# houkensjtu/taichi-2d-vof

Hardware: AMD Instinct MI355X
Metric: cell-updates/sec (whole node), 4096x4096 fp64 dam-break (higher is better)
Workload: dtype f64; 1 GPU; 4096x4096 -ic 1 f64, dt 4e-06, 10 Jacobi sweeps/step, single strip; nx=4096, ny=4096, jacobi_iters=10, exchange=none, tm_choice=1, step_schedule=k_tm batch graphs (k_transport + the next step's k_momentum as one kernel), handle_warm_steps=19

## Files before the change

### taichi-2d-vof_amd/csrc/kernels/jacobi_pair.h

```cpp
#pragma once
#include "jacobi.h"

namespace vof {

template <typename T, int V>
struct JpRing {
  static constexpr int W = 64 * V, NR = 8;
  T p[NR][W], b[NR][W];
  int hit;
};
template <typename T, int V>
__device__ __forceinline__ void jp_put(T (&row)[64 * V], int lane, const T (&c)[V]) {
  Pack<T, V> k;
#pragma unroll
  for (int q = 0; q < V; ++q) k.v[q] = c[q];
  *reinterpret_cast<Pack<T, V>*>(&row[lane * V]) = k;
}
template <typename T, int V>
__device__ __forceinline__ void jp_get(T (&c)[V], const T (&row)[64 * V], int lane) {
  const Pack<T, V> k = *reinterpret_cast<const Pack<T, V>*>(&row[lane * V]);
#pragma unroll
  for (int q = 0; q < V; ++q) c[q] = k.v[q];
}

template <typename T, int V, int TS, bool BS, int ROLE, int ABL = 0>
__device__ __forceinline__ void jacobi_pair_march(const Geom& g, const Consts<T>& c, const T* __restrict__ p,
                                                  const T* __restrict__ rhs, T* __restrict__ pn, JpRing<T, V>& lds,
                                                  int c0, int lane, int ra, int rb, WaveTimer& wt) {
  if constexpr ((ROLE == 0 && !(ABL & ABL_PRIO0)) || (ROLE == 1 && (ABL & ABL_PRIO1))) __builtin_amdgcn_s_setprio(1);
  constexpr int W = 64 * V;
  constexpr int H = ((2 * TS + V - 1) / V) * V;
  const int j0 = c0 + lane * V;
  const int nx = g.nx, ny = g.ny;
  const int jlo = c0 + H > 1 ? c0 + H : 1;
  const int jhi = c0 + W - H - 1 < ny ? c0 + W - H - 1 : ny;
  const int64_t pitch = g.pitch;
  T cj[V], apI[V], yI[V];
#pragma unroll
  for (int q = 0; q < V; ++q) {
    const int j = j0 + q;
    const T an = j != ny ? c.dyi2 : (T)0.0, as_ = j != 1 ? c.dyi2 : (T)0.0;
    cj[q] = (j >= 1 && j <= ny) ? c.dxi2 : (T)0.0;
    apI[q] = (T)-1.0 * (c.dxi2 + c.dxi2 + an + as_);
    yI[q] = (T)1 / apI[q];
    if (j < 1 || j > ny) yI[q] = (T)0;
  }
  auto rowptr = [&](const T* base, int r) {
    if constexpr ((ABL & ABL_FIXED_ROW) != 0) r = ra;
    const int rc = r < g.row_lo ? g.row_lo : (r > g.row_hi ? g.row_hi : r);
    return base + (size_t)(rc - g.row_lo) * (size_t)pitch + (size_t)(g.col0 + j0);
  };
  auto to_products = [&](T (&row)[V], int r) {
    const bool rowok = r >= 1 && r <= nx;
#pragma unroll
    for (int q = 0; q < V; ++q) row[q] = (rowok ? cj[q] : (T)0.0) * row[q];
  };
  T ring[TS][3][V];
  T rq[6][V];
#pragma unroll
  for (int s = 0; s < TS; ++s)
#pragma unroll
    for (int k = 0; k < 3; ++k)
#pragma unroll
      for (int q = 0; q < V; ++q) ring[s][k][q] = (T)0;
#pragma unroll
  for (int k = 0; k < 6; ++k)
#pragma unroll
    for (int q = 0; q < V; ++q) rq[k][q] = (T)0;
  const int t0 = ra - TS + 2, t1 = rb + TS;
  if constexpr (ROLE == 0) {
    load_c<T, V>(ring[0][0], rowptr(p, t0 - 2));
    load_c<T, V>(ring[0][1], rowptr(p, t0 - 1));
    load_c<T, V>(ring[0][2], rowptr(p, t0));
    load_s<T, V>(rq[0], rowptr(rhs, t0 - 1));
  } else {
    for (int k = 0; k < 2 * TS + 2; ++k) wt.barrier();
    jp_get<T, V>(ring[0][0], lds.p[(t0 - 2) & 7], lane);
    jp_get<T, V>(ring[0][1], lds.p[(t0 - 1) & 7], lane);
    jp_get<T, V>(ring[0][2], lds.p[t0 & 7], lane);
    jp_get<T, V>(rq[0], lds.b[(t0 - 1) & 7], lane);
  }
  to_products(ring[0][0], t0 - 2);
  to_products(ring[0][1], t0 - 1);
  const T* const pn_tile = pn + (int64_t)(g.col0 + c0);
  const int voff_st = (j0 >= jlo && j0 + V - 1 <= jhi) ? lane * (int)(V * sizeof(T)) : kBufSkip;
  const T* const p_tile = p + (int64_t)(g.col0 + c0);
  const T* const rhs_tile = rhs + ((int64_t)(g.col0 + c0) - pitch);
  const int voff_ld = lane * (int)(V * sizeof(T));
  int soff = 0;
  auto sub = [&](auto uc, auto fc, int t) {
    constexpr int U = decltype(uc)::value;
    constexpr bool FAST = decltype(fc)::value != 0;
    constexpr int kM = U % 3, kC = (U + 1) % 3, kE = (U + 2) % 3;
    T carry[V];
    if constexpr (ROLE == 1 && (ABL & ABL_IDLE1)) { wt.barrier(); return; }
    if constexpr (ROLE == 0) jp_put<T, V>(lds.b[(t - 1) & 7], lane, rq[U % 6]);
    if constexpr (ROLE == 0 && (ABL & ABL_PASS0)) {
      const int io = t - TS;
      if (io >= ra && io <= rb) jp_put<T, V>(lds.p[io & 7], lane, ring[0][kC]);
      if (t < t1) {
        load_c<T, V>(ring[0][kM], rowptr(p, t + 1));
        load_s<T, V>(rq[(U + 1) % 6], rowptr(rhs, t));
      }
      wt.barrier();
      return;
    }
    if constexpr (FAST) {
#pragma unroll
      for (int q = 0; q < V; ++q) ring[0][kE][q] = cj[q] * ring[0][kE][q];
    } else {
      to_products(ring[0][kE], t);
    }
#pragma unroll
    for (int s = 1; s <= TS; ++s) {
      const int i = t - s;
      const T sl = lane_up_z(ring[s - 1][kC][V - 1]);
      const T sr = lane_dn_z(ring[s - 1][kC][0]);
      if (s > 1) {
        const T coef = (FAST || (i + 1 >= 1 && i + 1 <= nx)) ? c.dxi2 : (T)0.0;
#pragma unroll
        for (int q = 0; q < V; ++q) ring[s - 1][kE][q] = coef * carry[q];
      }
      if (!FAST && s > 1 && t < ra - TS + 2 * s) continue;
      const bool edge = !FAST && ((i == 1) || (i == nx));
      const int slot = ((U + 1 - s) % 6 + 6) % 6;
      T num[V];
#pragma unroll
      for (int q = 0; q < V; ++q) {
        const T N = q == V - 1 ? sr : ring[s - 1][kC][q + 1];
        const T S = q == 0 ? sl : ring[s - 1][kC][q - 1];
        num[q] = rq[slot][q] - ring[s - 1][kE][q] - ring[s - 1][kM][q] - N - S;
      }
      if (edge) {
        const T ae = i != nx ? c.dxi2 : (T)0.0;
        const T aw = i != 1 ? c.dxi2 : (T)0.0;
#pragma unroll
        for (int q = 0; q < V; ++q) {
          int j = j0 + q;
          asm volatile("" : "+v"(j));
          const T an = j != ny ? c.dyi2 : (T)0.0, as_ = j != 1 ? c.dyi2 : (T)0.0;
          const T ap = (T)-1.0 * (ae + aw + an + as_);
          T o = div_by_const<T>(num[q], ap, (T)1.0 / ap);
          if (j < 1 || j > ny) o = (T)0;
          carry[q] = o;
        }
      } else {
        div_by_const_v<T, V, false, ColdFlagLds>(carry, num, apI, yI, ColdFlagLds{&lds.hit});
      }
      if (s == 1) {
        if constexpr (FAST) {
          if constexpr (ROLE == 0) {
            load_buf<T, V>(ring[0][kM], p_tile, voff_ld, soff, false);
            load_buf<T, V>(rq[(U + 1) % 6], rhs_tile, voff_ld, soff, true);
            if constexpr ((ABL & ABL_FIXED_ROW) == 0) soff += (int)(pitch * (int64_t)sizeof(T));
          } else {
            jp_get<T, V>(ring[0][kM], lds.p[(t + 1) & 7], lane);
            jp_get<T, V>(rq[(U + 1) % 6], lds.b[t & 7], lane);
          }
        } else if (t < t1) {
          if constexpr (ROLE == 0) {
            load_c<T, V>(ring[0][kM], rowptr(p, t + 1));
            load_s<T, V>(rq[(U + 1) % 6], rowptr(rhs, t));
          } else {
            jp_get<T, V>(ring[0][kM], lds.p[(t + 1) & 7], lane);
            jp_get<T, V>(rq[(U + 1) % 6], lds.b[t & 7], lane);
          }
        }
      }
    }
    const int io = t - TS;
    if constexpr (ROLE == 0) {
      if (FAST || (io >= ra && io <= rb)) jp_put<T, V>(lds.p[io & 7], lane, carry);
    } else if constexpr ((ABL & ABL_NO_STORE) != 0) {
      asm volatile("" :: "v"(carry[0]), "v"(carry[V - 1]));
    } else if constexpr (BS) {
      if constexpr (FAST) {
        store_buf_nt<T, V>(pn_tile, voff_st, soff, carry);
        soff += (int)(pitch * (int64_t)sizeof(T));
      } else {
        store_buf_nt<T, V>(pn_tile, (io >= ra && io <= rb) ? voff_st : kBufSkip,
                           (io >= ra && io <= rb) ? (int)((int64_t)(io - g.row_lo) * pitch * (int64_t)sizeof(T)) : 0, carry);
      }
    } else if (FAST || (io >= ra && io <= rb)) {
      store_s<T, V>(pn + at(g, io, j0), carry, j0, jlo, jhi);
    }
    wt.barrier();
  };
  auto imax3 = [](int a, int b, int d) { return a > b ? (a > d ? a : d) : (b > d ? b : d); };
  auto imin3 = [](int a, int b, int d) { return a < b ? (a < d ? a : d) : (b < d ? b : d); };
  const int fast_lo = imax3(ra + TS, TS + 2, g.row_lo + TS);
  const int fast_hi = imin3(nx - 1, t1 - 1, g.row_hi - 1);
  int t = t0;
  bool done = false;
  for (int phase = 0; phase < 2; ++phase) {
    for (; !done && t <= t1 && (phase == 1 || t < fast_lo || t + 5 > fast_hi); t += 6) {
      sub(IC<0>{}, IC<0>{}, t);
      if (t + 1 > t1) { done = true; break; }
      sub(IC<1>{}, IC<0>{}, t + 1);
      if (t + 2 > t1) { done = true; break; }
      sub(IC<2>{}, IC<0>{}, t + 2);
      if (t + 3 > t1) { done = true; break; }
      sub(IC<3>{}, IC<0>{}, t + 3);
      if (t + 4 > t1) { done = true; break; }
      sub(IC<4>{}, IC<0>{}, t + 4);
      if (t + 5 > t1) { done = true; break; }
      sub(IC<5>{}, IC<0>{}, t + 5);
    }
    if (BS && phase == 0 && !done && t <= t1 && t >= fast_lo && t + 5 <= fast_hi) {
      soff = (int)((int64_t)((ROLE == 0 ? t + 1 : t - TS) - g.row_lo) * pitch * (int64_t)sizeof(T));
      for (; t + 5 <= fast_hi; t += 6) {
        sub(IC<0>{}, IC<1>{}, t);
        sub(IC<1>{}, IC<1>{}, t + 1);
        sub(IC<2>{}, IC<1>{}, t + 2);
        sub(IC<3>{}, IC<1>{}, t + 3);
        sub(IC<4>{}, IC<1>{}, t + 4);
        sub(IC<5>{}, IC<1>{}, t + 5);
      }
    }
  }
  if constexpr (ROLE == 0) { wt.barrier(); wt.barrier(); }
}

template <typename T, int V, int TS, bool BS, int ABL = 0>
__global__ __launch_bounds__(128) __attribute__((amdgpu_waves_per_eu(4))) void k_jacobi_pair(Geom g, Consts<T> c, const T* __restrict__ p,
                                                     const T* __restrict__ rhs, T* __restrict__ pn, int R, int ntt,
                                                     TbPlan tp, int first, int last) {
  constexpr int W = 64 * V;
  constexpr int H = ((2 * TS + V - 1) / V) * V;
  constexpr int STRIDE = W - 2 * H;
  __shared__ __attribute__((aligned(16))) JpRing<T, V> lds;
  WaveTimer wt_(WT_JACOBI_PAIR);
  if (last < first) { first = g.ilo; last = g.ihi; }
  const int pair = (int)blockIdx.x;
  const int role = __builtin_amdgcn_readfirstlane(threadIdx.x >> 6);
  const int lane = threadIdx.x & 63;
  int upair;
  upair = xcd_grouped_block(pair, (int)gridDim.x);
  int tj = upair % ntt, ra = first + (upair / ntt) * R, rb = ra + R - 1;
  bool planned = false;
  if (tp.masks != nullptr) {
    const unsigned long long* pl = tp.plan;
    if (pl[0] == plan_key(tp)) {
      const unsigned long long e = pl[1 + pair];
      tj = (int)(e & 0xffull);
      ra = (int)((e >> 8) & 0xfffffffull);
      rb = (int)((e >> 36) & 0xfffffffull);
      planned = true;
    }
  }
  tj = __builtin_amdgcn_readfirstlane(tj);
  ra = __builtin_amdgcn_readfirstlane(ra);
  rb = __builtin_amdgcn_readfirstlane(rb);
  if (planned && rb < ra) return;
  if (planned && ra < first) ra = first;
  if (ra > last) return;
  if (rb > last) rb = last;
  if (rb < ra) return;
  const int c0 = 1 - H + tj * STRIDE;
  if (threadIdx.x == 0) lds.hit = 0;
  __syncthreads();
  if (role == 0) {
    jacobi_pair_march<T, V, TS, BS, 0, ABL>(g, c, p, rhs, pn, lds, c0, lane, ra - TS, rb + TS, wt_);
  } else {
    jacobi_pair_march<T, V, TS, BS, 1, ABL>(g, c, p, rhs, pn, lds, c0, lane, ra, rb, wt_);
  }
  if (tp.masks != nullptr) {
    __syncthreads();
    if (threadIdx.x == 0 && lds.hit != 0) {
      for (int b = tb_band_of(g, ra < g.ilo ? g.ilo : ra); b <= tb_band_of(g, rb > g.ihi ? g.ihi : rb); ++b)
        atomicOr(tp.masks + tb_word(tp.par ^ 1, b, tj), 1ull << (tj & 63));
    }
  }
}

}
```

### taichi-2d-vof_amd/csrc/runtime/context.h

```cpp
#pragma once
#include <vector>

#include <float.h>
#include <hip/hip_runtime.h>
#include <hip/hip_ext.h>
#include <dlfcn.h>

#include <cmath>
#include <cstdio>
#include <cstdlib>
#include <cstring>
#include <map>
#include <new>

#include "../../../include/vof2d.h"
#include "../vof2d_kernels.h"

using namespace vof;

struct RcclId { char internal[VOF_COMM_ID_BYTES]; };

namespace {

enum FieldId { fF = 0, fF2, fU, fV, fP, fPT, fUS, fVS, fMX, fMY, fKAPPA, fRHO, fNU, fRHS, NFIELDS };
// ... 162 lines not shown
  double* mg_sc = nullptr;
  int mg_nu = 2;
  int mg_levels = -1;
  int mg_graph = 1;
  void* mg_key[3] = {nullptr, nullptr, nullptr};
  int mg_coarse_block = 0;
  double* mg_rec = nullptr;
  void* step_mg_key[NFIELDS] = {};
  int step_mg_cycles = 0, step_mg_crit = 0;
  double* diag_part = nullptr;
  double* diag_rows = nullptr;
  int64_t diag_cap = 0;
  int rows_override = 0;
  int tb = 5;
  int tb_rows = 0;
  int mom_rows = 0;
  int tb_general = 0;
  int tb_adapt = 1;
  unsigned long long* d_tbmask = nullptr;
  long tbplan_cap = 0;
  int fctx_rows = 0;
  int fctx_corr_rows = 0;
  int fuse_transport = 1;
  int band_rows = 4;
  int buf_stores = 7;
  int virtual_ghosts = 1;
  void* f_home = nullptr;
  void* us_home = nullptr;
  void* p_home = nullptr;
  int phase_graph_ori = 0;
  GraphCache graphs;
  static constexpr int kStepBatches = GraphCache::kStepBatches;
  static constexpr int kTuneBatch = 1;
  int step_batch[kStepBatches] = {16, 8, 2};
  int fuse_tm = -1;
  double gas_share = -1.0;
  unsigned long long* h_gas = nullptr;
  hipEvent_t ev_gas = nullptr;
  bool gas_pending = false;
  bool tm_broken = false;
  bool alt_dirty = false;
  bool ahead = false;
  bool tm_rhs_alt = false;
  int64_t tm_chained = 0;
  int jpair = 1;
  int jpair_rows = 0;
  int solve_pairs = -1;
  int pair_slow10 = 32;
  int tb_slow10 = 20;
  int pair_vec4 = 0;
  bool jpair_active = false;
  bool jpair_captured = false;
  int64_t pair_launches = 0;
  TuneState tune;
  int64_t tm_steps = 0;
  int tm_rows = 0;
  int halves = -1;
  std::vector<hipStream_t> chain_streams;
  bool halves_captured[kStepBatches] = {};
  int64_t halves_steps = 0;
  std::vector<hipEvent_t> hev;
  bool batching = true;
  int next_phase = 0;
  bool f_ghosts_dirty = true;
  bool uv_ghosts_dirty = false;
  bool ghosts_virtual = false;
  void* vis = nullptr;
  size_t vis_bytes = 0;
  static constexpr int kMaxTimed = 96;
  hipEvent_t tev[2 * kMaxTimed] = {};
  int timed = -1;
  int tkid[kMaxTimed];
  double prof_sum_ms[24] = {};
  long prof_cnt[24] = {};
  std::map<const void*, long> occ_cache;
  void* comm = nullptr;
  hipStream_t cstream = nullptr;
  hipEvent_t ev_ready = nullptr, ev_done = nullptr;
  hipEvent_t ev_fork[3] = {nullptr, nullptr, nullptr};
  int xchg5_graph = 1;
  int xchg_pair = 1;
  int xchg_graph = 1;
  int64_t xchg_steps = 0;
  int64_t xchg_graph_steps = 0;
  double* d_red = nullptr;
  int comm_rank = 0, comm_world = 1;
  int peer_lo = -1, peer_hi = -1;
  char err[512];
};

namespace {

#define HIPCHK(h, call)                                                                          \
  do {                                                                                           \
    hipError_t e_ = (call);                                                                      \
    if (e_ != hipSuccess) {                                                                      \
      snprintf((h)->err, sizeof((h)->err), "%s:%d %s -> %s", __FILE__, __LINE__, #call,          \
               hipGetErrorString(e_));                                                           \
      return VOF_EHIP;                                                                           \
    }                                                                                            \
  } while (0)

int fail(vof2d_ctx* h, int code, const char* msg) {
  if (h) snprintf(h->err, sizeof(h->err), "%s", msg);
  return code;
}
// ... 12 lines not shown
```

### taichi-2d-vof_amd/csrc/runtime/launches.h

```cpp
#pragma once
#include "context.h"

namespace {

template <typename K>
long resident_blocks(vof2d_ctx* h, K kernel, int threads) {
  std::map<const void*, long>& cache = h->occ_cache;
  const void* key = reinterpret_cast<const void*>(kernel);
  auto it = cache.find(key);
  if (it != cache.end()) return it->second;
  int blocks_per_cu = 0;
  long cap = 6L * 256;
  if (hipOccupancyMaxActiveBlocksPerMultiprocessor(&blocks_per_cu, kernel, threads, 0) == hipSuccess && blocks_per_cu > 0) {
    int cus = 256;
    hipDeviceProp_t prop;
    if (hipGetDeviceProperties(&prop, h->device) == hipSuccess && prop.multiProcessorCount > 0) cus = prop.multiProcessorCount;
    cap = (long)blocks_per_cu * cus;
  } else {
    (void)hipGetLastError();
  }
  cache[key] = cap;
  return cap;
}
template <typename K>
// ... 136 lines not shown
           (const T*)F_<T>(h, fRHO), (const T*)F_<T>(h, fNU), F_<T>(h, fUS), F_<T>(h, fVS), R);
  }
  static void momentum(vof2d_ctx* h, bool virt = false, int adapt_par = -1, int first = 1, int last = 0) {
    constexpr int Wt = 64 * V, Ht = TileHalo::momentum, ST = Wt - 2 * Ht;
    const int ntt = (h->g.ny + ST - 1) / ST;
    if (last < first) { first = h->g.ilo; last = h->g.ihi; }
    const bool bs = buffer_stores_ok(h) && (h->buf_stores & 1);
    int R = h->mom_rows > 0 ? h->mom_rows : chunk_rows_fit(h, ntt, bs ? resident_waves(h, k_momentum<T, V, true>) : resident_waves(h, k_momentum<T, V, false>), 4, 64);
    if (h->mom_rows <= 0 && R > 32) R = 14;
    const TbPlan tp = tb_plan(h, adapt_par);
    const unsigned mom_blocks = blocks_rows(last - first + 1, ntt, R);
    if (bs)
      launch(h, kMomentum, k_momentum<T, V, true>, dim3(mom_blocks + (tp.masks ? 1u : 0u)), 0, h->g, C(h), (const T*)F_<T>(h, fF),
             (const T*)F_<T>(h, fU), (const T*)F_<T>(h, fV), F_<T>(h, fUS), F_<T>(h, fVS), F_<T>(h, fRHS), R, ntt,
             virt ? 1 : 0, tp, first, last);
    else
      launch(h, kMomentum, k_momentum<T, V, false>, dim3(mom_blocks + (tp.masks ? 1u : 0u)), 0, h->g, C(h), (const T*)F_<T>(h, fF),
             (const T*)F_<T>(h, fU), (const T*)F_<T>(h, fV), F_<T>(h, fUS), F_<T>(h, fVS), F_<T>(h, fRHS), R, ntt,
             virt ? 1 : 0, tp, first, last);
  }
  template <bool STORED>
  static void rhs(vof2d_ctx* h) {
    const int R = pick_rows(h, h->g.ntj);
    launch(h, kRhs, k_rhs<T, V, STORED>, dim3(blocks_for(h, h->g.ntj, R)), 0, h->g, C(h), (const T*)F_<T>(h, fUS),
           (const T*)F_<T>(h, fVS), (const T*)F_<T>(h, fF), (const T*)F_<T>(h, fRHO), F_<T>(h, fRHS), R);
  }
  template <bool RESID>
  static void jacobi(vof2d_ctx* h, int src, int dst) {
    const int R = pick_rows(h, h->g.ntj);
    launch(h, kJacobi, k_jacobi<T, V, 2, RESID>, dim3(blocks_for(h, h->g.ntj, R)), 0, h->g, C(h),
           (const T*)F_<T>(h, src), (const T*)F_<T>(h, fRHS), F_<T>(h, dst), R, h->d_courant + 1);
  }
  template <int TS, int VV>
  static int jacobi_tb_plan(vof2d_ctx* h, bool sq, int& ntt) {
    constexpr int Wt = 64 * VV;
    const int Ht = ((TS - 1 + (sq ? 1 : 0) + VV - 1) / VV) * VV, ST = Wt - 2 * Ht;
    ntt = (h->g.ny + ST - 1) / ST;
    const long cap = sq ? resident_waves(h, k_jacobi_tb<T, VV, TS, true, false>) : resident_waves(h, k_jacobi_tb<T, VV, TS, false, false>);
    return h->tb_rows > 0 ? h->tb_rows : chunk_rows_fit(h, ntt, cap, 4, 96);
  }
  static bool jacobi_pair_ok(vof2d_ctx* h) {
    const Consts<T> cc = C(h);
    return h->jpair >= 1 && cc.dxi2 == cc.dyi2 && !h->tb_general && h->tb >= 5 &&
           h->d.jacobi_iters % 10 == 0;
  }
  static int pair_vec(const vof2d_ctx* h) {
#ifdef VOF_PAIR_VEC4
    return (sizeof(T) == 4 && h->pair_vec4 && h->g.ny % 4 == 0 && buffer_stores_ok(h)) ? 4 : V;
#else
    (void)h;
    return V;
#endif
  }
  template <int VV>
  static int jacobi_pair_geom_v(vof2d_ctx* h, int& ntt) {
    constexpr int ST = 64 * VV - 2 * (((2 * 5 + VV - 1) / VV) * VV);
    ntt = (h->g.ny + ST - 1) / ST;
    const bool bs = buffer_stores_ok(h) && (h->buf_stores & 2);
    const long cap = bs ? resident_blocks(h, k_jacobi_pair<T, VV, 5, true>, 128) : resident_blocks(h, k_jacobi_pair<T, VV, 5, false>, 128);
    return h->jpair_rows > 0 ? h->jpair_rows : chunk_rows_fit(h, ntt, cap, 8, 160);
  }
  static int jacobi_pair_geom(vof2d_ctx* h, int& ntt) {
#ifdef VOF_PAIR_VEC4
    if constexpr (sizeof(T) == 4) { if (pair_vec(h) == 4) return jacobi_pair_geom_v<4>(h, ntt); }
#endif
    return jacobi_pair_geom_v<V>(h, ntt);
  }
  template <int VV>
  static void jacobi_pair_v(vof2d_ctx* h, int src, int dst, int adapt_par, int first, int last) {
    int ntt = 0;
    const int R = jacobi_pair_geom_v<VV>(h, ntt);
    const TbPlan tp = tb_plan(h, adapt_par);
    const unsigned pairs = tp.masks ? (unsigned)tp.waves : (unsigned)(((last - first + R) / R) * ntt);
    const bool bs = buffer_stores_ok(h) && (h->buf_stores & 2);
    if (bs)
      launch_block(h, kJacobiPair, k_jacobi_pair<T, VV, 5, true>, dim3(pairs), 128u, 0, h->g, C(h), (const T*)F_<T>(h, src),
                   (const T*)F_<T>(h, fRHS), F_<T>(h, dst), R, ntt, tp, first, last);
    else
      launch_block(h, kJacobiPair, k_jacobi_pair<T, VV, 5, false>, dim3(pairs), 128u, 0, h->g, C(h), (const T*)F_<T>(h, src),
                   (const T*)F_<T>(h, fRHS), F_<T>(h, dst), R, ntt, tp, first, last);
  }
  static void jacobi_pair(vof2d_ctx* h, int src, int dst, int adapt_par = -1, int first = 1, int last = 0) {
    if (last < first) { first = h->g.ilo; last = h->g.ihi; }
#ifdef VOF_PAIR_VEC4
    if constexpr (sizeof(T) == 4) { if (pair_vec(h) == 4) return jacobi_pair_v<4>(h, src, dst, adapt_par, first, last); }
#endif
    jacobi_pair_v<V>(h, src, dst, adapt_par, first, last);
  }
  static TbPlan tb_plan(vof2d_ctx* h, int adapt_par) {
    TbPlan tp{nullptr, nullptr, 0, 0, 0, 0, 0};
    if (adapt_par < 0 || !h->tb_adapt || h->tb < 5 || h->tb_rows > 0) return tp;
    const Consts<T> cc = C(h);
    const bool sq = cc.dxi2 == cc.dyi2 && !h->tb_general;
    int ntt = 0;
    int R;
    long waves;
    if (h->jpair_active) {
      R = jacobi_pair_geom(h, ntt);
      waves = (long)((h->g.ihi - h->g.ilo + R) / R) * ntt;
    } else {
      R = jacobi_tb_plan<5, V>(h, sq, ntt);
      waves = (long)blocks_for(h, ntt, R) * 4;
    }
    if (ntt > TB_COLS || waves > kTbPlanWaves) return tp;
    tp.masks = h->d_tbmask;
    tp.plan = h->d_tbmask + 2 * TB_BANDS * (TB_COLS / 64);
    tp.ntt = ntt; tp.R = R; tp.waves = (int)waves; tp.par = adapt_par;
    tp.slow10 = h->jpair_active ? h->pair_slow10 : h->tb_slow10;
    return tp;
  }
  template <int TS, int VV>
  static void jacobi_tb_launch(vof2d_ctx* h, const Consts<T>& cc, bool sq, int src, int dst, int R, int ntt, int adapt_par = -1,
                               int first = 1, int last = 0) {
    if (last < first) { first = h->g.ilo; last = h->g.ihi; }

    unsigned long long* none = nullptr;
    TbPlan tp{nullptr, nullptr, 0, 0, 0, 0, 0};
    if (TS == 5 && VV == V) tp = tb_plan(h, adapt_par);
    const unsigned nblk = tp.masks ? blocks_for(h, ntt, R) : blocks_rows(last - first + 1, ntt, R);
    const bool one_round = (long)blocks_for(h, ntt, R) * 4 <= resident_waves(h, k_jacobi_tb<T, VV, TS, true, false>);
    constexpr bool kBufForm = sizeof(T) * VV == 16 || sizeof(T) * VV == 8;
    if (kBufForm && sq && one_round && buffer_stores_ok(h) && (h->buf_stores & 2)) {
      if constexpr (kBufForm)
        launch(h, kJacobiTB, k_jacobi_tb<T, VV, TS, true, false, true>, dim3(nblk), 0, h->g, cc,
               (const T*)F_<T>(h, src), (const T*)F_<T>(h, fRHS), F_<T>(h, dst), R, ntt, none, tp, first, last);
    } else if (sq)
      launch(h, kJacobiTB, k_jacobi_tb<T, VV, TS, true, false>, dim3(nblk), 0, h->g, cc,
// ... 210 lines not shown
```

### taichi-2d-vof_amd/csrc/runtime/schedule.h

```cpp
#pragma once
#include "graphs.h"

namespace {

void swap_F(vof2d_ctx* h) {
  void* t = h->fld[fF];
  h->fld[fF] = h->fld[fF2];
  h->fld[fF2] = t;
}

template <typename T, bool POST, bool CORR = false>
void sweep_x(vof2d_ctx* h) { L<T>::template fct_x<POST, CORR>(h); swap_F(h); }
template <typename T, bool POST, bool CORR = false>
void sweep_y(vof2d_ctx* h) { L<T>::template fct_y<POST, CORR>(h); swap_F(h); }
template <typename T>
void final_sweep(vof2d_ctx* h, bool along_x) {
  const int lo = h->d.own_lo > h->g.ilo ? h->d.own_lo : h->g.ilo, hi = h->d.own_hi < h->g.ihi ? h->d.own_hi : h->g.ihi;
  if (hi < lo) return;
  if (along_x) L<T>::template fct_x<true, false>(h, lo, hi); else L<T>::template fct_y<true, false>(h, lo, hi);
}

enum TransportPart { kAllOwned = 0, kEdgeBands = 1, kRest = 2 };
template <typename T>
void transport_part(vof2d_ctx* h, bool y_first, int part) {
// ... 170 lines not shown
    h->stream = st[0];
    for (int p = 0; p < P - 1; ++p) s[p] -= kHalvesDrift;
    ++n;
  };
  for (int k = 0; k < K && ok; ++k) {
    const int64_t istep = first_step + k;
    const int par = (int)(istep & 1);
    if (k > 0) {
      for (int p = 1; p < P - 1; ++p) ok = ok && hipStreamWaitEvent(st[0], ev_done[p * total + n_lastjac], 0) == hipSuccess;
      ok = ok && hipStreamWaitEvent(st[0], ev_plan[k - 1], 0) == hipSuccess;
    }
    const int n_mom = n;
    all([&](int a, int b, bool first) { L<T>::momentum(h, true, first ? par : -1, a, b); });
    for (int p = 2; p < P; ++p) ok = ok && hipStreamWaitEvent(st[p], ev_done[n_mom], 0) == hipSuccess;
    int cur = fP, oth = fPT;
    for (int j = 0; j < nj; ++j) {
      all([&](int a, int b, bool) { L<T>::template jacobi_tb<5>(h, cur, oth, par, a, b); });
      const int t = cur; cur = oth; oth = t;
    }
    n_lastjac = n - 1;
    ok = ok && hipEventRecord(ev_plan[k], st[P - 1]) == hipSuccess;
    all([&](int a, int b, bool) {
      const RowRanges rr{{a, 1, 1}, {b, 0, 0}, {L<T>::transport_rows(h), 1, 1}};
      if (istep % 2 == 0) L<T>::template transport<true>(h, &rr); else L<T>::template transport<false>(h, &rr);
    });
    swap_F(h);
  }
  for (int p = 1; p < P; ++p)
    ok = ok && hipEventRecord(ev_join[p - 1], st[p]) == hipSuccess && hipStreamWaitEvent(st[0], ev_join[p - 1], 0) == hipSuccess;
  return ok;
}

inline void swap_P(vof2d_ctx* h) { void* t = h->fld[fP]; h->fld[fP] = h->fld[fPT]; h->fld[fPT] = t; }
template <typename T>
void batch_jacobi(vof2d_ctx* h, int par) {
  const int nj = h->d.jacobi_iters / 5;
  if (L<T>::jacobi_pair_ok(h)) {
    for (int j = 0; j < nj / 2; ++j) {
      L<T>::jacobi_pair(h, fP, fPT, par);
      swap_P(h);
    }
    return;
  }
  int cur = fP, oth = fPT;
  for (int j = 0; j < nj; ++j) {
    L<T>::template jacobi_tb<5>(h, cur, oth, par);
    const int t = cur; cur = oth; oth = t;
  }
}
template <typename T>
void enqueue_steps_tm(vof2d_ctx* h, int64_t first_step, int K) {
  h->jpair_active = L<T>::jacobi_pair_ok(h);
  h->jpair_captured = h->jpair_active;
  h->tm_rhs_alt = true;
  for (int k = 0; k < K; ++k) {
    const int64_t istep = first_step + k;
    const int par = (int)(istep & 1);
    batch_jacobi<T>(h, par);
    if (k < K - 1) {
      if (istep % 2 == 0) L<T>::template tm<true, false>(h, par ^ 1); else L<T>::template tm<false, false>(h, par ^ 1);
    } else {
      if (istep % 2 == 0) L<T>::template tm<true, true>(h, par ^ 1); else L<T>::template tm<false, true>(h, par ^ 1);
    }
    swap_SR(h);
    swap_F(h);
  }
  h->tm_rhs_alt = false;
  if (h->jpair_active && ((K * (h->d.jacobi_iters / 10)) & 1)) swap_P(h);
  h->jpair_active = false;
}
template <typename T>
void enqueue_tm_head(vof2d_ctx* h, int par) {
  h->jpair_active = L<T>::jacobi_pair_ok(h);
  L<T>::momentum(h, true, par);
  h->jpair_active = false;
}
int settle_ahead(vof2d_ctx* h) {
  if (!h->ahead) return VOF_OK;
  h->ahead = false;
  auto copy = [&](int dst, int src, int i0, int j0) -> hipError_t {
    const size_t pitch = (size_t)h->g.pitch * h->esz;
    const size_t off = ((size_t)(i0 - h->d.row_lo) * h->g.pitch + h->g.col0 + j0) * h->esz;
    return hipMemcpy2DAsync(reinterpret_cast<char*>(h->fld[dst]) + off, pitch, reinterpret_cast<const char*>(h->fld[src]) + off, pitch,
                            (size_t)(h->g.ny - j0 + 1) * h->esz, (size_t)(h->g.nx - i0 + 1), hipMemcpyDeviceToDevice, h->stream);
  };
  HIPCHK(h, copy(fUS, fMX, 2, 1));
  HIPCHK(h, copy(fVS, fMY, 1, 2));
  HIPCHK(h, copy(fRHS, fKAPPA, 1, 1));
  return VOF_OK;
}

int ensure_ok(vof2d_ctx* h) {
  hipError_t e = hipGetLastError();
  if (e != hipSuccess) {
    snprintf(h->err, sizeof(h->err), "kernel launch failed: %s", hipGetErrorString(e));
    return VOF_EHIP;
  }
  return VOF_OK;
}

#define DISPATCH_T(h, expr_d, expr_f) \
  do { if ((h)->d.dtype == VOF_F64) { expr_d; } else { expr_f; } } while (0)
#define DISPATCH_B(h, expr_d, expr_f) ((h)->d.dtype == VOF_F64 ? (expr_d) : (expr_f))

bool step_leaves_ghosts_virtual(const vof2d_ctx* h) {
  return h->g.wall_lo && h->g.wall_hi && h->fuse_transport &&
// ... 55 lines not shown
```

### taichi-2d-vof_amd/csrc/runtime/step.h

```cpp
#pragma once
#include "schedule.h"
#include "multigrid.h"

namespace {

bool post_gas_count(vof2d_ctx* h) {
  hipStreamCaptureStatus cs = hipStreamCaptureStatusNone;
  if (hipStreamIsCapturing(h->stream, &cs) != hipSuccess || cs != hipStreamCaptureStatusNone) { (void)hipGetLastError(); return false; }
  if (!h->h_gas && hipHostMalloc(reinterpret_cast<void**>(&h->h_gas), sizeof(unsigned long long), hipHostMallocDefault) != hipSuccess) { (void)hipGetLastError(); h->h_gas = nullptr; return false; }
  if (!h->ev_gas && hipEventCreateWithFlags(&h->ev_gas, hipEventDisableTiming) != hipSuccess) { (void)hipGetLastError(); h->ev_gas = nullptr; return false; }
  unsigned long long* cnt = h->d_courant + 3;
  bool ok = hipMemsetAsync(cnt, 0, sizeof(*cnt), h->stream) == hipSuccess;
  const unsigned blocks = (unsigned)(h->g.ihi - h->g.ilo + 1 < 2048 ? h->g.ihi - h->g.ilo + 1 : 2048);
  if (h->d.dtype == VOF_F64) hipLaunchKernelGGL(k_gas_cells<double>, dim3(blocks), dim3(256), 0, h->stream, h->g, (const double*)F_<double>(h, fF), cnt);
  else hipLaunchKernelGGL(k_gas_cells<float>, dim3(blocks), dim3(256), 0, h->stream, h->g, (const float*)F_<float>(h, fF), cnt);
  ok = ok && hipMemcpyAsync(h->h_gas, cnt, sizeof(*cnt), hipMemcpyDeviceToHost, h->stream) == hipSuccess;
  ok = ok && hipEventRecord(h->ev_gas, h->stream) == hipSuccess;
  if (!ok) (void)hipGetLastError();
  h->gas_pending = ok;
  return ok;
}
void decide_batch_form_by_rule(vof2d_ctx* h) {
  if (!h->gas_pending && !post_gas_count(h)) return;
  h->gas_pending = false;
// ... 59 lines not shown
          h->halves_captured[b] = true;
          DISPATCH_T(h, enq = enqueue_steps_halves<double>(h, first, K), enq = enqueue_steps_halves<float>(h, first, K));
        } else if (variant) DISPATCH_T(h, enqueue_steps_tm<double>(h, first, K), enqueue_steps_tm<float>(h, first, K));
        else
          for (int k = 0; k < K; ++k)
            DISPATCH_T(h, enqueue_step<double>(h, first + k, true, true), enqueue_step<float>(h, first + k, true, true));
        return enq;
      }) == hipSuccess;
    }
    if (c) swap_F(h);
  }
  if (!ok) {
    (void)hipGetLastError();
    GraphCache::clear(&GB[0][0][0], &GB[0][0][0] + vof2d_ctx::kStepBatches * 4);
    if (variant) h->tm_broken = true; else h->batching = false;
    if (getenv("VOF2D_DEBUG")) fprintf(stderr, "[vof2d] step batches (%s) could not be captured: %s\n", variant ? "k_tm form" : "chains / plain",
                                       variant ? "the other form stays" : "one graph launch per step");
  }
}

int run_step_batch(vof2d_ctx* h, int64_t remaining, int* ran) {
  *ran = 0;
  const int par = (int)(h->istep & 1), ori = ori_F(h);
  bool timed = false;
  int variant = batch_form(h, true, remaining, &timed);
  if (h->batching && !h->graphs.batch[variant][0][par][ori]) {
    build_step_batches(h, variant);
    if (variant && h->tm_broken) {
      variant = 0; timed = false;
      if (h->batching && !h->graphs.batch[0][0][par][ori]) build_step_batches(h, 0);
    }
  }
  auto& GB = h->graphs.batch[variant];
  TuneState& t = h->tune;
  for (int b = timed ? vof2d_ctx::kTuneBatch : 0; b < vof2d_ctx::kStepBatches; ++b) {
    const int K = batch_steps(h, variant, b);
    if (remaining < K || !GB[b][par][ori]) continue;
    const bool time_it = timed && b == vof2d_ctx::kTuneBatch && h->batching;
    if (time_it) {
      for (int k = 0; k < 2; ++k)
        if (!t.ev[2 * t.n + k] && hipEventCreate(&t.ev[2 * t.n + k]) != hipSuccess) return fail(h, VOF_EHIP, "hipEventCreate");
      if (hipEventRecord(t.ev[2 * t.n], h->stream) != hipSuccess) return fail(h, VOF_EHIP, "hipEventRecord");
    }
    if (variant) {
      if (h->ahead) h->tm_chained += 1;
      else DISPATCH_T(h, enqueue_tm_head<double>(h, par), enqueue_tm_head<float>(h, par));
      h->ahead = true;
    } else h->ahead = false;
    if (hipGraphLaunch(GB[b][par][ori], h->stream) != hipSuccess) return fail(h, VOF_EHIP, "hipGraphLaunch of a step batch");
    if (time_it) {
      if (hipEventRecord(t.ev[2 * t.n + 1], h->stream) == hipSuccess) t.n += 1;
      else (void)hipGetLastError();
    }
    if (variant) { h->tm_steps += K; if (h->jpair_captured) h->pair_launches += (int64_t)K * (h->d.jacobi_iters / 10); }
    else if (h->halves_captured[b]) h->halves_steps += K;
    *ran = K;
    return VOF_OK;
  }
  return VOF_OK;
}
int run_step_graph(vof2d_ctx* h, bool virt) {
  hipGraphExec_t& exec = h->graphs.step[(int)(h->istep & 1)][ori_F(h)];
  int rc;
  if (!exec && (rc = capture_or_fail(h, true, &exec, "the step graph", [&] {
        DISPATCH_T(h, enqueue_step<double>(h, h->istep, true, virt), enqueue_step<float>(h, h->istep, true, virt));
      })))
    return rc;
  HIPCHK(h, hipGraphLaunch(exec, h->stream));
  if (h->g.wall_lo && h->g.wall_hi && h->fuse_transport) swap_F(h);
  return VOF_OK;
}
int run_step_eager(vof2d_ctx* h, bool lean, bool virt) {
  DISPATCH_T(h, enqueue_step<double>(h, h->istep, lean, virt), enqueue_step<float>(h, h->istep, lean, virt));
  return ensure_ok(h);
}

int step_n(vof2d_ctx* h, int64_t nsteps) {
  const bool use_graph = !(h->d.flags & VOF_FLAG_NO_GRAPH);
  for (int64_t s = 0; s < nsteps; ++s) {
    h->istep += 1;
    const bool lean = !h->f_ghosts_dirty;
    const bool virt = step_leaves_ghosts_virtual(h);
    if (!virt) settle_ghosts(h);
    const bool captured = use_graph && lean && !h->uv_ghosts_dirty;
    int rc, ran = 0;
    if (captured && virt) {
      if ((rc = run_step_batch(h, nsteps - s, &ran))) { h->istep -= 1; return rc; }
      if (ran) {
        h->istep += ran - 1;
        s += ran - 1;
        h->ghosts_virtual = true;
        continue;
      }
    }
    h->ahead = false;
    if ((rc = captured ? run_step_graph(h, virt) : run_step_eager(h, lean, virt))) return rc;
    h->f_ghosts_dirty = false;
    h->uv_ghosts_dirty = false;
    h->ghosts_virtual = virt;
  }
  return VOF_OK;
}

int run_step_mg_graph(vof2d_ctx* h, bool virt, const StepMg& mg) {
  GraphCache& G = h->graphs;
  void* key[NFIELDS];
  memcpy(key, h->fld, sizeof(key));
// ... 130 lines not shown
```

### taichi-2d-vof_amd/csrc/vof2d_api.hip

```cpp
#include "runtime/context.h"
#include "runtime/launches.h"
#include "runtime/graphs.h"
#include "runtime/schedule.h"
#include "runtime/multigrid.h"
#include "runtime/step.h"
#include "runtime/diag_reduce.h"
#include "runtime/comm.h"
#include "runtime/selftest.h"
#ifdef VOF_WAVE_TIMES
#include "runtime/diag.h"
#endif

namespace {

struct Knob { const char* name; int* (*at)(vof2d_ctx*); bool readable; };
#define KNOB(name, member, readable) {name, [](vof2d_ctx* h) { return &h->member; }, readable}
const Knob kKnobs[] = {
  KNOB("jacobi_tb", tb, true), KNOB("jacobi_tb_adapt", tb_adapt, true), KNOB("jacobi_tb_rows", tb_rows, false),
  KNOB("jacobi_tb_general", tb_general, false), KNOB("momentum_rows", mom_rows, false), KNOB("fctx_rows", fctx_rows, false),
  KNOB("fctx_corr_rows", fctx_corr_rows, false), KNOB("band_rows", band_rows, false), KNOB("rows_per_wave", rows_override, false),
  KNOB("fuse_transport", fuse_transport, false), KNOB("virtual_ghosts", virtual_ghosts, false), KNOB("buffer_stores", buf_stores, false),
  KNOB("overlap_halves", halves, false), KNOB("batch_steps", step_batch[0], false), KNOB("fuse_tm", fuse_tm, false),
  KNOB("tm_rows", tm_rows, false), KNOB("jacobi_pair", jpair, false), KNOB("jacobi_pair_rows", jpair_rows, false),
  KNOB("pair_vec4", pair_vec4, false), KNOB("pair_slow10", pair_slow10, false), KNOB("solve_pairs", solve_pairs, false),
// ... 551 lines not shown
  if (!h || !name || !value) return VOF_EINVAL;
#define P(n) if (!strcmp(name, #n)) { *value = h->cd.n; return VOF_OK; }
  P(sigma) P(dt) P(dx) P(dy) P(dxi) P(dyi) P(dxi2) P(dyi2) P(rho_l) P(rho_g) P(nu_l) P(nu_g) P(gx) P(gy)
  P(nrm_x) P(nrm_y) P(kap_x) P(kap_y) P(dxdy) P(dtdy) P(dtdx) P(cfl_x) P(cfl_y) P(half_dx) P(half_dy)
  P(sqrt2dx) P(tiny)
#undef P
  if (!strcmp(name, "Lx")) { *value = h->d.Lx; return VOF_OK; }
  if (!strcmp(name, "Ly")) { *value = h->d.Ly; return VOF_OK; }
  if (!strcmp(name, "pitch")) { *value = (double)h->g.pitch; return VOF_OK; }
  if (!strcmp(name, "rows_per_wave")) { *value = (double)pick_rows(h, h->g.ntj); return VOF_OK; }
  if (!strcmp(name, "overlap_halves")) { *value = halves_eligible(h, h->step_batch[vof2d_ctx::kTuneBatch]) ? 1.0 : 0.0; return VOF_OK; }
  if (!strcmp(name, "gas_share")) { *value = h->gas_share; return VOF_OK; }
  if (!strcmp(name, "fuse_transport")) {
    *value = (h->g.wall_lo && h->g.wall_hi && h->fuse_transport) ? 1.0 : 0.0;
    return VOF_OK;
  }
  if (!strcmp(name, "mg_coarse_block")) { *value = mg_block_in_effect(h) ? 1.0 : 0.0; return VOF_OK; }
  if (const Knob* k = find_knob(name))
    if (k->readable) { *value = (double)*k->at(h); return VOF_OK; }
  return fail(h, VOF_EINVAL, "unknown parameter");
}
int vof_get_counter(vof2d_handle h, const char* name, int64_t* value) {
  if (!h || !name || !value) return VOF_EINVAL;
  if (!strcmp(name, "courant_violations")) {
    unsigned long long v = 0;
    HIPCHK(h, hipMemcpyAsync(&v, h->d_courant, sizeof(v), hipMemcpyDeviceToHost, h->stream));
    HIPCHK(h, hipStreamSynchronize(h->stream));
    *value = (int64_t)v;
    return VOF_OK;
  }
  if (!strcmp(name, "tb_plan_active")) {
    unsigned long long v = 0;
    HIPCHK(h, hipMemcpyAsync(&v, h->d_tbmask + 2 * TB_BANDS * (TB_COLS / 64), sizeof(v), hipMemcpyDeviceToHost, h->stream));
    HIPCHK(h, hipStreamSynchronize(h->stream));
    *value = v ? 1 : 0;
    return VOF_OK;
  }
#ifdef VOF_WAVE_TIMES
  if (!strncmp(name, "dbg_plan_", 9)) {
    unsigned long long v = 0;
    HIPCHK(h, hipMemcpyAsync(&v, h->d_tbmask + 2 * TB_BANDS * (TB_COLS / 64), sizeof(v), hipMemcpyDeviceToHost, h->stream));
    HIPCHK(h, hipStreamSynchronize(h->stream));
    h->jpair_active = true;
    const TbPlan tp = L<double>::tb_plan(h, (int)(h->istep & 1));
    h->jpair_active = false;
    *value = !strcmp(name, "dbg_plan_word") ? (int64_t)v : !strcmp(name, "dbg_plan_waves") ? tp.waves : !strcmp(name, "dbg_plan_R") ? tp.R : tp.ntt;
    return VOF_OK;
  }
#endif
  if (!strcmp(name, "pair_launches")) {
    *value = h->pair_launches;
    return VOF_OK;
  }
  if (!strcmp(name, "tm_chained_batches")) {
    *value = h->tm_chained;
    return VOF_OK;
  }
  if (!strcmp(name, "tm_steps")) {
    *value = h->tm_steps;
    return VOF_OK;
  }
  if (!strcmp(name, "tm_choice")) {
    *value = ((tm_auto(h) || tm_by_rule(h)) && h->tune.decided) ? h->tune.choice : -1;
    return VOF_OK;
  }
  if (!strcmp(name, "halves_steps")) {
    *value = h->halves_steps;
    return VOF_OK;
  }
  if (!strcmp(name, "exchange_graph_steps")) {
    *value = h->xchg_graph_steps;
    return VOF_OK;
  }
  return fail(h, VOF_EINVAL, "unknown counter");
}

int vof_sync(vof2d_handle h) {
  if (!h) return VOF_EINVAL;
  HIPCHK(h, hipStreamSynchronize(h->stream));
  return ensure_ok(h);
}
int vof_timer_start(vof2d_handle h) {
  if (!h) return VOF_EINVAL;
  HIPCHK(h, hipEventRecord(h->ev0, h->stream));
  return VOF_OK;
}
int vof_timer_stop(vof2d_handle h, float* ms) {
  if (!h || !ms) return VOF_EINVAL;
  HIPCHK(h, hipEventRecord(h->ev1, h->stream));
  HIPCHK(h, hipEventSynchronize(h->ev1));
  HIPCHK(h, hipEventElapsedTime(ms, h->ev0, h->ev1));
  return VOF_OK;
}
int vof_profile_steps(vof2d_handle h, int64_t nsteps) {
  if (!h) return VOF_EINVAL;
  if (nsteps < 0) return fail(h, VOF_EINVAL, "nsteps must be >= 0");
  if (h->next_phase != 0) return fail(h, VOF_ESTATE, "a phased step (vof_step_phase) is in progress");
  return profile_steps(h, nsteps);
}
int vof_get_profile(vof2d_handle h, const char* kernel, double* avg_us, int64_t* launches) {
  if (!h || !kernel) return VOF_EINVAL;
  for (int k = 0; k < NKERNELS; ++k)
    if (!strcmp(kernel, kKernelNames[k])) {
      if (avg_us) *avg_us = h->prof_cnt[k] ? 1e3 * h->prof_sum_ms[k] / (double)h->prof_cnt[k] : 0.0;
      if (launches) *launches = h->prof_cnt[k];
      return VOF_OK;
// ... 150 lines not shown
```

Before: 41.47 billion cell-updates/s.

## Add DMA-to-LDS prefetch path for the jacobi pair producer wave

Adds an optional path in which the producer wave of the Jacobi pair kernel streams p and rhs rows straight into LDS with global_load_lds, several rows ahead. The rhs ring grows to 16 slots, and the per-step barrier waits on a bounded vmcnt so loads stay in flight. The aim is to take global-load latency and register staging off the producer's critical path. The cost is more LDS per block and a lower waves_per_eu hint (3 instead of 4). The path is only chosen when jacobi_pair is set to 3, and adds a launch counter for it.

New measurement: 40.68 billion cell-updates/s. 1.9% lower.

```diff
diff --git a/taichi-2d-vof_amd/csrc/kernels/jacobi_pair.h b/taichi-2d-vof_amd/csrc/kernels/jacobi_pair.h
--- a/taichi-2d-vof_amd/csrc/kernels/jacobi_pair.h
+++ b/taichi-2d-vof_amd/csrc/kernels/jacobi_pair.h
@@ -3,12 +3,14 @@
 
 namespace vof {
 
-template <typename T, int V>
+template <typename T, int V, bool DMA = false>
 struct JpRing {
   static constexpr int W = 64 * V, NR = 8;
-  T p[NR][W], b[NR][W];
+  static constexpr int NB = DMA ? 16 : NR;
+  T p[NR][W], b[NB][W];
   int hit;
 };
+constexpr int JP_LEAD = 3, JP_PSLOT = 4;
 template <typename T, int V>
 __device__ __forceinline__ void jp_put(T (&row)[64 * V], int lane, const T (&c)[V]) {
   Pack<T, V> k;
@@ -23,10 +25,46 @@
   for (int q = 0; q < V; ++q) c[q] = k.v[q];
 }
 
-template <typename T, int V, int TS, bool BS, int ROLE, int ABL = 0>
+template <typename T, int V, bool NT>
+__device__ __forceinline__ void jp_dma(T (&row)[64 * V], const T* src, int lane) {
+  typedef const __attribute__((address_space(1))) void* gptr;
+  typedef __attribute__((address_space(3))) void* lptr;
+  if constexpr (sizeof(T) * V == 16) {
+    __builtin_amdgcn_global_load_lds((gptr)(src + lane * V), (lptr)&row[0], 16, 0, NT ? 2 : 0);
+  } else {
+    static_assert(sizeof(T) == 4, "4 bytes per lane and request");
+#pragma unroll
+    for (int k = 0; k < V; ++k) __builtin_amdgcn_global_load_lds((gptr)(src + 64 * k + lane), (lptr)&row[64 * k], 4, 0, NT ? 2 : 0);
+  }
+}
+template <typename T, int V>
+constexpr int jp_dma_per_step = 2 * (sizeof(T) * V == 16 ? 1 : V);
+template <int N>
+__device__ __forceinline__ void jp_dma_barrier(WaveTimer& wt) {
+  asm volatile("s_waitcnt vmcnt(%0)" ::"n"(N) : "memory");
+#ifdef VOF_WAVE_TIMES
+  const unsigned long long tb = wt.on ? __builtin_readcyclecounter() : 0ull;
+#endif
+  asm volatile("s_waitcnt lgkmcnt(0)" ::: "memory");
+  __builtin_amdgcn_s_barrier();
+  asm volatile("" ::: "memory");
+#ifdef VOF_WAVE_TIMES
+  if (wt.on) wt.wait += __builtin_readcyclecounter() - tb;
+#else
+  (void)wt;
+#endif
+}
+
+template <typename T, int V, int TS, bool BS, int ROLE, int ABL = 0, bool DMA = false>
 __device__ __forceinline__ void jacobi_pair_march(const Geom& g, const Consts<T>& c, const T* __restrict__ p,
-                                                  const T* __restrict__ rhs, T* __restrict__ pn, JpRing<T, V>& lds,
+                                                  const T* __restrict__ rhs, T* __restrict__ pn, JpRing<T, V, DMA>& lds,
                                                   int c0, int lane, int ra, int rb, WaveTimer& wt) {
+  static_assert(!DMA || ABL == 0, "the ablated forms are forms of the register path");
+  constexpr int MB = JpRing<T, V, DMA>::NB - 1;
+  constexpr int kFlight = (JP_LEAD - 2) * jp_dma_per_step<T, V>;
+  auto step_barrier = [&]() {
+    if constexpr (DMA && ROLE == 0) jp_dma_barrier<kFlight>(wt); else wt.barrier();
+  };
   if constexpr ((ROLE == 0 && !(ABL & ABL_PRIO0)) || (ROLE == 1 && (ABL & ABL_PRIO1))) __builtin_amdgcn_s_setprio(1);
   constexpr int W = 64 * V;
   constexpr int H = ((2 * TS + V - 1) / V) * V;
@@ -50,6 +88,10 @@
     const int rc = r < g.row_lo ? g.row_lo : (r > g.row_hi ? g.row_hi : r);
     return base + (size_t)(rc - g.row_lo) * (size_t)pitch + (size_t)(g.col0 + j0);
   };
+  auto rowbase = [&](const T* base, int r) {
+    const int rc = r < g.row_lo ? g.row_lo : (r > g.row_hi ? g.row_hi : r);
+    return base + (size_t)(rc - g.row_lo) * (size_t)pitch + (size_t)(g.col0 + c0);
+  };
   auto to_products = [&](T (&row)[V], int r) {
     const bool rowok = r >= 1 && r <= nx;
 #pragma unroll
@@ -73,19 +115,26 @@
     load_c<T, V>(ring[0][1], rowptr(p, t0 - 1));
     load_c<T, V>(ring[0][2], rowptr(p, t0));
     load_s<T, V>(rq[0], rowptr(rhs, t0 - 1));
+    if constexpr (DMA) {
+      for (int r = t0; r < t0 + JP_LEAD; ++r) {
+        jp_dma<T, V, false>(lds.b[(r + JP_PSLOT) & MB], rowbase(p, r), lane);
+        jp_dma<T, V, true>(lds.b[r & MB], rowbase(rhs, r), lane);
+      }
+      step_barrier();
+    }
   } else {
-    for (int k = 0; k < 2 * TS + 2; ++k) wt.barrier();
+    for (int k = 0; k < 2 * TS + 2 + (DMA ? 1 : 0); ++k) wt.barrier();
     jp_get<T, V>(ring[0][0], lds.p[(t0 - 2) & 7], lane);
     jp_get<T, V>(ring[0][1], lds.p[(t0 - 1) & 7], lane);
     jp_get<T, V>(ring[0][2], lds.p[t0 & 7], lane);
-    jp_get<T, V>(rq[0], lds.b[(t0 - 1) & 7], lane);
+    jp_get<T, V>(rq[0], lds.b[(t0 - 1) & MB], lane);
   }
   to_products(ring[0][0], t0 - 2);
   to_products(ring[0][1], t0 - 1);
   const T* const pn_tile = pn + (int64_t)(g.col0 + c0);
   const int voff_st = (j0 >= jlo && j0 + V - 1 <= jhi) ? lane * (int)(V * sizeof(T)) : kBufSkip;
   const T* const p_tile = p + (int64_t)(g.col0 + c0);
-  const T* const rhs_tile = rhs + ((int64_t)(g.col0 + c0) - pitch);
+  const T* const rhs_tile = rhs + ((int64_t)(g.col0 + c0) - (DMA ? 0 : pitch));
   const int voff_ld = lane * (int)(V * sizeof(T));
   int soff = 0;
   auto sub = [&](auto uc, auto fc, int t) {
@@ -94,7 +143,7 @@
     constexpr int kM = U % 3, kC = (U + 1) % 3, kE = (U + 2) % 3;
     T carry[V];
     if constexpr (ROLE == 1 && (ABL & ABL_IDLE1)) { wt.barrier(); return; }
-    if constexpr (ROLE == 0) jp_put<T, V>(lds.b[(t - 1) & 7], lane, rq[U % 6]);
+    if constexpr (ROLE == 0 && !DMA) jp_put<T, V>(lds.b[(t - 1) & 7], lane, rq[U % 6]);
     if constexpr (ROLE == 0 && (ABL & ABL_PASS0)) {
       const int io = t - TS;
       if (io >= ra && io <= rb) jp_put<T, V>(lds.p[io & 7], lane, ring[0][kC]);
@@ -148,14 +197,27 @@
         div_by_const_v<T, V, false, ColdFlagLds>(carry, num, apI, yI, ColdFlagLds{&lds.hit});
       }
       if (s == 1) {
-        if constexpr (FAST) {
+        if constexpr (DMA && ROLE == 0) {
+          if (FAST || t < t1) {
+            jp_get<T, V>(ring[0][kM], lds.b[(t + 1 + JP_PSLOT) & MB], lane);
+            jp_get<T, V>(rq[(U + 1) % 6], lds.b[t & MB], lane);
+          }
+          if constexpr (FAST) {
+            jp_dma<T, V, false>(lds.b[(t + JP_LEAD + JP_PSLOT) & MB], (const T*)((const char*)p_tile + soff), lane);
+            jp_dma<T, V, true>(lds.b[(t + JP_LEAD) & MB], (const T*)((const char*)rhs_tile + soff), lane);
+            soff += (int)(pitch * (int64_t)sizeof(T));
+          } else {
+            jp_dma<T, V, false>(lds.b[(t + JP_LEAD + JP_PSLOT) & MB], rowbase(p, t + JP_LEAD), lane);
+            jp_dma<T, V, true>(lds.b[(t + JP_LEAD) & MB], rowbase(rhs, t + JP_LEAD), lane);
+          }
+        } else if constexpr (FAST) {
           if constexpr (ROLE == 0) {
             load_buf<T, V>(ring[0][kM], p_tile, voff_ld, soff, false);
             load_buf<T, V>(rq[(U + 1) % 6], rhs_tile, voff_ld, soff, true);
             if constexpr ((ABL & ABL_FIXED_ROW) == 0) soff += (int)(pitch * (int64_t)sizeof(T));
           } else {
             jp_get<T, V>(ring[0][kM], lds.p[(t + 1) & 7], lane);
-            jp_get<T, V>(rq[(U + 1) % 6], lds.b[t & 7], lane);
+            jp_get<T, V>(rq[(U + 1) % 6], lds.b[t & MB], lane);
           }
         } else if (t < t1) {
           if constexpr (ROLE == 0) {
@@ -163,7 +225,7 @@
             load_s<T, V>(rq[(U + 1) % 6], rowptr(rhs, t));
           } else {
             jp_get<T, V>(ring[0][kM], lds.p[(t + 1) & 7], lane);
-            jp_get<T, V>(rq[(U + 1) % 6], lds.b[t & 7], lane);
+            jp_get<T, V>(rq[(U + 1) % 6], lds.b[t & MB], lane);
           }
         }
       }
@@ -184,12 +246,12 @@
     } else if (FAST || (io >= ra && io <= rb)) {
       store_s<T, V>(pn + at(g, io, j0), carry, j0, jlo, jhi);
     }
-    wt.barrier();
+    step_barrier();
   };
   auto imax3 = [](int a, int b, int d) { return a > b ? (a > d ? a : d) : (b > d ? b : d); };
   auto imin3 = [](int a, int b, int d) { return a < b ? (a < d ? a : d) : (b < d ? b : d); };
   const int fast_lo = imax3(ra + TS, TS + 2, g.row_lo + TS);
-  const int fast_hi = imin3(nx - 1, t1 - 1, g.row_hi - 1);
+  const int fast_hi = imin3(nx - 1, t1 - 1, g.row_hi - (DMA && ROLE == 0 ? JP_LEAD : 1));
   int t = t0;
   bool done = false;
   for (int phase = 0; phase < 2; ++phase) {
@@ -207,7 +269,7 @@
       sub(IC<5>{}, IC<0>{}, t + 5);
     }
     if (BS && phase == 0 && !done && t <= t1 && t >= fast_lo && t + 5 <= fast_hi) {
-      soff = (int)((int64_t)((ROLE == 0 ? t + 1 : t - TS) - g.row_lo) * pitch * (int64_t)sizeof(T));
+      soff = (int)((int64_t)((ROLE == 0 ? t + (DMA ? JP_LEAD : 1) : t - TS) - g.row_lo) * pitch * (int64_t)sizeof(T));
       for (; t + 5 <= fast_hi; t += 6) {
         sub(IC<0>{}, IC<1>{}, t);
         sub(IC<1>{}, IC<1>{}, t + 1);
@@ -218,17 +280,18 @@
       }
     }
   }
+  if constexpr (DMA && ROLE == 0) asm volatile("s_waitcnt vmcnt(0)" ::: "memory");
   if constexpr (ROLE == 0) { wt.barrier(); wt.barrier(); }
 }
 
-template <typename T, int V, int TS, bool BS, int ABL = 0>
-__global__ __launch_bounds__(128) __attribute__((amdgpu_waves_per_eu(4))) void k_jacobi_pair(Geom g, Consts<T> c, const T* __restrict__ p,
+template <typename T, int V, int TS, bool BS, int ABL = 0, bool DMA = false>
+__global__ __launch_bounds__(128) __attribute__((amdgpu_waves_per_eu(DMA ? 3 : 4))) void k_jacobi_pair(Geom g, Consts<T> c, const T* __restrict__ p,
                                                      const T* __restrict__ rhs, T* __restrict__ pn, int R, int ntt,
                                                      TbPlan tp, int first, int last) {
   constexpr int W = 64 * V;
   constexpr int H = ((2 * TS + V - 1) / V) * V;
   constexpr int STRIDE = W - 2 * H;
-  __shared__ __attribute__((aligned(16))) JpRing<T, V> lds;
+  __shared__ __attribute__((aligned(16))) JpRing<T, V, DMA> lds;
   WaveTimer wt_(WT_JACOBI_PAIR);
   if (last < first) { first = g.ilo; last = g.ihi; }
   const int pair = (int)blockIdx.x;
@@ -260,9 +323,9 @@
   if (threadIdx.x == 0) lds.hit = 0;
   __syncthreads();
   if (role == 0) {
-    jacobi_pair_march<T, V, TS, BS, 0, ABL>(g, c, p, rhs, pn, lds, c0, lane, ra - TS, rb + TS, wt_);
+    jacobi_pair_march<T, V, TS, BS, 0, ABL, DMA>(g, c, p, rhs, pn, lds, c0, lane, ra - TS, rb + TS, wt_);
   } else {
-    jacobi_pair_march<T, V, TS, BS, 1, ABL>(g, c, p, rhs, pn, lds, c0, lane, ra, rb, wt_);
+    jacobi_pair_march<T, V, TS, BS, 1, ABL, DMA>(g, c, p, rhs, pn, lds, c0, lane, ra, rb, wt_);
   }
   if (tp.masks != nullptr) {
     __syncthreads();
diff --git a/taichi-2d-vof_amd/csrc/runtime/context.h b/taichi-2d-vof_amd/csrc/runtime/context.h
--- a/taichi-2d-vof_amd/csrc/runtime/context.h
+++ b/taichi-2d-vof_amd/csrc/runtime/context.h
@@ -238,6 +238,8 @@
   bool jpair_active = false;
   bool jpair_captured = false;
   int64_t pair_launches = 0;
+  bool jpair_dma_captured = false;
+  int64_t pair_dma_launches = 0;
   TuneState tune;
   int64_t tm_steps = 0;
   int tm_rows = 0;
diff --git a/taichi-2d-vof_amd/csrc/runtime/launches.h b/taichi-2d-vof_amd/csrc/runtime/launches.h
--- a/taichi-2d-vof_amd/csrc/runtime/launches.h
+++ b/taichi-2d-vof_amd/csrc/runtime/launches.h
@@ -212,12 +212,18 @@
     return V;
 #endif
   }
+  static bool pair_dma(const vof2d_ctx* h) {
+    if (pair_vec(h) != V) return false;
+    return h->jpair == 3;
+  }
   template <int VV>
   static int jacobi_pair_geom_v(vof2d_ctx* h, int& ntt) {
     constexpr int ST = 64 * VV - 2 * (((2 * 5 + VV - 1) / VV) * VV);
     ntt = (h->g.ny + ST - 1) / ST;
     const bool bs = buffer_stores_ok(h) && (h->buf_stores & 2);
-    const long cap = bs ? resident_blocks(h, k_jacobi_pair<T, VV, 5, true>, 128) : resident_blocks(h, k_jacobi_pair<T, VV, 5, false>, 128);
+    long cap;
+    if (VV == V && pair_dma(h)) cap = bs ? resident_blocks(h, k_jacobi_pair<T, V, 5, true, 0, true>, 128) : resident_blocks(h, k_jacobi_pair<T, V, 5, false, 0, true>, 128);
+    else cap = bs ? resident_blocks(h, k_jacobi_pair<T, VV, 5, true>, 128) : resident_blocks(h, k_jacobi_pair<T, VV, 5, false>, 128);
     return h->jpair_rows > 0 ? h->jpair_rows : chunk_rows_fit(h, ntt, cap, 8, 160);
   }
   static int jacobi_pair_geom(vof2d_ctx* h, int& ntt) {
@@ -233,6 +239,18 @@
     const TbPlan tp = tb_plan(h, adapt_par);
     const unsigned pairs = tp.masks ? (unsigned)tp.waves : (unsigned)(((last - first + R) / R) * ntt);
     const bool bs = buffer_stores_ok(h) && (h->buf_stores & 2);
+    if (VV == V && pair_dma(h)) {
+      hipStreamCaptureStatus cs = hipStreamCaptureStatusNone;
+      if (hipStreamIsCapturing(h->stream, &cs) != hipSuccess) (void)hipGetLastError();
+      else if (cs == hipStreamCaptureStatusNone) h->pair_dma_launches += 1;
+      if (bs)
+        launch_block(h, kJacobiPair, k_jacobi_pair<T, V, 5, true, 0, true>, dim3(pairs), 128u, 0, h->g, C(h), (const T*)F_<T>(h, src),
+                     (const T*)F_<T>(h, fRHS), F_<T>(h, dst), R, ntt, tp, first, last);
+      else
+        launch_block(h, kJacobiPair, k_jacobi_pair<T, V, 5, false, 0, true>, dim3(pairs), 128u, 0, h->g, C(h), (const T*)F_<T>(h, src),
+                     (const T*)F_<T>(h, fRHS), F_<T>(h, dst), R, ntt, tp, first, last);
+      return;
+    }
     if (bs)
       launch_block(h, kJacobiPair, k_jacobi_pair<T, VV, 5, true>, dim3(pairs), 128u, 0, h->g, C(h), (const T*)F_<T>(h, src),
                    (const T*)F_<T>(h, fRHS), F_<T>(h, dst), R, ntt, tp, first, last);
diff --git a/taichi-2d-vof_amd/csrc/runtime/schedule.h b/taichi-2d-vof_amd/csrc/runtime/schedule.h
--- a/taichi-2d-vof_amd/csrc/runtime/schedule.h
+++ b/taichi-2d-vof_amd/csrc/runtime/schedule.h
@@ -246,6 +246,7 @@
 void enqueue_steps_tm(vof2d_ctx* h, int64_t first_step, int K) {
   h->jpair_active = L<T>::jacobi_pair_ok(h);
   h->jpair_captured = h->jpair_active;
+  h->jpair_dma_captured = h->jpair_active && L<T>::pair_dma(h);
   h->tm_rhs_alt = true;
   for (int k = 0; k < K; ++k) {
     const int64_t istep = first_step + k;
diff --git a/taichi-2d-vof_amd/csrc/runtime/step.h b/taichi-2d-vof_amd/csrc/runtime/step.h
--- a/taichi-2d-vof_amd/csrc/runtime/step.h
+++ b/taichi-2d-vof_amd/csrc/runtime/step.h
@@ -135,7 +135,7 @@
       if (hipEventRecord(t.ev[2 * t.n + 1], h->stream) == hipSuccess) t.n += 1;
       else (void)hipGetLastError();
     }
-    if (variant) { h->tm_steps += K; if (h->jpair_captured) h->pair_launches += (int64_t)K * (h->d.jacobi_iters / 10); }
+    if (variant) { h->tm_steps += K; if (h->jpair_captured) h->pair_launches += (int64_t)K * (h->d.jacobi_iters / 10); if (h->jpair_dma_captured) h->pair_dma_launches += (int64_t)K * (h->d.jacobi_iters / 10); }
     else if (h->halves_captured[b]) h->halves_steps += K;
     *ran = K;
     return VOF_OK;
diff --git a/taichi-2d-vof_amd/csrc/vof2d_api.hip b/taichi-2d-vof_amd/csrc/vof2d_api.hip
--- a/taichi-2d-vof_amd/csrc/vof2d_api.hip
+++ b/taichi-2d-vof_amd/csrc/vof2d_api.hip
@@ -627,6 +627,10 @@
     *value = h->pair_launches;
     return VOF_OK;
   }
+  if (!strcmp(name, "jacobi_pair_dma_launches")) {
+    *value = h->pair_dma_launches;
+    return VOF_OK;
+  }
   if (!strcmp(name, "tm_chained_batches")) {
     *value = h->tm_chained;
     return VOF_OK;
```
